# AzureLeon1/DiffSpectra

Hardware: AMD Instinct MI355X
Metric: molecules/sec, 1000-step QM9S all-spectra sampling (partial run) (higher is better)
Workload: dtype f32 (GEMMs as split-fp16 x3 MFMA with fp32 accumulate; fp32-level accuracy, parity gates unchanged)

## Files before the change

diffspectra_amd/csrc/ds_device.h:

```cpp
#pragma once
#include <hip/hip_runtime.h>
#include <stdint.h>

typedef float f32x16 __attribute__((ext_vector_type(16)));
typedef float f32x2 __attribute__((ext_vector_type(2)));
typedef _Float16 h4 __attribute__((ext_vector_type(4)));
typedef _Float16 h8 __attribute__((ext_vector_type(8)));
typedef float f32x4 __attribute__((ext_vector_type(4)));

#define DS_LDP 4

__device__ __forceinline__ float ds_silu(float x) { return __fdividef(x, 1.0f + __expf(-x)); }
__device__ __forceinline__ float ds_tanh(float x) {
  const float e = __builtin_amdgcn_exp2f(x * 2.8853900817779268f);
  return fmaf(-2.0f, __builtin_amdgcn_rcpf(e + 1.0f), 1.0f);
}
__device__ __forceinline__ f32x2 ds_tanh2_prescaled(f32x2 t) {
  f32x2 e;
  e.x = __builtin_amdgcn_exp2f(t.x); e.y = __builtin_amdgcn_exp2f(t.y);
  const f32x2 d = e + 1.0f;
  f32x2 r;
  r.x = __builtin_amdgcn_rcpf(d.x); r.y = __builtin_amdgcn_rcpf(d.y);
  return r * -2.0f + 1.0f;
}
// ... 235 lines not shown
      }
    }
    __builtin_amdgcn_sched_barrier(0);
#pragma unroll
    for (int m = 0; m < MT; ++m) {
      if (TRANS) {
        hi[m] = __builtin_amdgcn_mfma_f32_32x32x16_f16(w1, xa[m][0], hi[m], 0, 0, 0);
        lo[m] = __builtin_amdgcn_mfma_f32_32x32x16_f16(w1, xa[m][1], lo[m], 0, 0, 0);
        lo[m] = __builtin_amdgcn_mfma_f32_32x32x16_f16(w2, xa[m][0], lo[m], 0, 0, 0);
      } else {
        hi[m] = __builtin_amdgcn_mfma_f32_32x32x16_f16(xa[m][0], w1, hi[m], 0, 0, 0);
        lo[m] = __builtin_amdgcn_mfma_f32_32x32x16_f16(xa[m][1], w1, lo[m], 0, 0, 0);
        lo[m] = __builtin_amdgcn_mfma_f32_32x32x16_f16(xa[m][0], w2, lo[m], 0, 0, 0);
      }
    }
    w1 = w1n; w2 = w2n;
#pragma unroll
    for (int m = 0; m < MT; ++m) {
      if (XPF) { xa[m][0] = xn[m][0]; xa[m][1] = xn[m][1]; }
      else {
        xa[m][0] = *reinterpret_cast<const h8*>(xr + m * 32 * ldh + kn * 16);
        xa[m][1] = *reinterpret_cast<const h8*>(xr + m * 32 * ldh + K_tile + kn * 16);
      }
    }
  }
}
constexpr int DS_MMA_XD = 1;
template <int PF>
struct WRingH {
  h8 w1[PF], w2[PF];
};
template <int PF>
__device__ __forceinline__ void wring_h(WRingH<PF>& ring, const WStreamH& ws, int kb0) {
#pragma unroll
  for (int i = 0; i < PF; ++i) {
    ring.w1[i] = wload_h(ws, 0, kb0 + i); ring.w2[i] = wload_h(ws, 1, kb0 + i);
    __builtin_amdgcn_sched_barrier(0);
  }
}
template <int MT, bool TRANS, int NKB, int PF, int XD = DS_MMA_XD>
__device__ __forceinline__ void wave_mma_h_deep(const _Float16* X, int K_tile, const WStreamH& ws, WRingH<PF>& ring, int kb0,
                                                f32x16 (&hi)[MT], f32x16 (&lo)[MT], int xkb0 = 0) {
  static_assert(PF <= NKB && XD <= NKB, "ring deeper than the product");
  const int lane = threadIdx.x & 63, r = lane & 31, hh = lane >> 5;
  const int ldh = 2 * K_tile + 8;
  const _Float16* xr = X + r * ldh + 8 * hh + (kb0 - xkb0) * 16;
  h8 xq[XD][MT][2];
#pragma unroll
  for (int d = 0; d < XD; ++d)
#pragma unroll
    for (int m = 0; m < MT; ++m) {
      xq[d][m][0] = *reinterpret_cast<const h8*>(xr + m * 32 * ldh + d * 16);
      xq[d][m][1] = *reinterpret_cast<const h8*>(xr + m * 32 * ldh + K_tile + d * 16);
    }
#pragma unroll
  for (int i = 0; i < NKB; ++i) {
    __builtin_amdgcn_sched_barrier(0);
    const h8 w1 = ring.w1[i % PF], w2 = ring.w2[i % PF];
    h8 xa[MT][2];
#pragma unroll
    for (int m = 0; m < MT; ++m) { xa[m][0] = xq[i % XD][m][0]; xa[m][1] = xq[i % XD][m][1]; }
#define DS_MMA_(ACC, WV, XV) ACC = TRANS ? __builtin_amdgcn_mfma_f32_32x32x16_f16(WV, XV, ACC, 0, 0, 0) : __builtin_amdgcn_mfma_f32_32x32x16_f16(XV, WV, ACC, 0, 0, 0)
#pragma unroll
    for (int m = 0; m < MT; ++m) DS_MMA_(lo[m], w1, xa[m][1]);
#pragma unroll
    for (int m = 0; m < MT; ++m) DS_MMA_(hi[m], w1, xa[m][0]);
#pragma unroll
    for (int m = 0; m < MT; ++m) DS_MMA_(lo[m], w2, xa[m][0]);
#undef DS_MMA_
    if (i + PF < NKB) {
      ring.w1[i % PF] = wload_h(ws, 0, kb0 + i + PF);
      ring.w2[i % PF] = wload_h(ws, 1, kb0 + i + PF);
    }
    if (i + XD < NKB) {
#pragma unroll
      for (int m = 0; m < MT; ++m) {
        xq[i % XD][m][0] = *reinterpret_cast<const h8*>(xr + m * 32 * ldh + (i + XD) * 16);
        xq[i % XD][m][1] = *reinterpret_cast<const h8*>(xr + m * 32 * ldh + K_tile + (i + XD) * 16);
      }
    }
    __builtin_amdgcn_sched_barrier(0);
  }
}
template <int MT, bool TRANS, int NKB, int PF>
__device__ __forceinline__ void wave_mma_h_deep_t2(const _Float16* X, int K_tile, const WStreamH& wsA, const WStreamH& wsB,
                                                   WRingH<PF>& ringA, WRingH<PF>& ringB, int kb0, f32x16 (&hiA)[MT], f32x16 (&loA)[MT],
                                                   f32x16 (&hiB)[MT], f32x16 (&loB)[MT], int xkb0 = 0) {
  static_assert(PF <= NKB, "ring deeper than the product");
  const int lane = threadIdx.x & 63, r = lane & 31, hh = lane >> 5;
  const int ldh = 2 * K_tile + 8;
  const _Float16* xr = X + r * ldh + 8 * hh + (kb0 - xkb0) * 16;
  h8 xa[MT][2];
#pragma unroll
  for (int m = 0; m < MT; ++m) {
    xa[m][0] = *reinterpret_cast<const h8*>(xr + m * 32 * ldh);
    xa[m][1] = *reinterpret_cast<const h8*>(xr + m * 32 * ldh + K_tile);
  }
#define DS_MMA_(ACC, WV, XV) ACC = TRANS ? __builtin_amdgcn_mfma_f32_32x32x16_f16(WV, XV, ACC, 0, 0, 0) : __builtin_amdgcn_mfma_f32_32x32x16_f16(XV, WV, ACC, 0, 0, 0)
#pragma unroll
  for (int i = 0; i < NKB; ++i) {
    const int in = i + 1 < NKB ? i + 1 : i;
    h8 xn[MT][2];
#pragma unroll
    for (int m = 0; m < MT; ++m) {
      xn[m][0] = *reinterpret_cast<const h8*>(xr + m * 32 * ldh + in * 16);
      xn[m][1] = *reinterpret_cast<const h8*>(xr + m * 32 * ldh + K_tile + in * 16);
    }
    __builtin_amdgcn_sched_barrier(0);
    const h8 a1 = ringA.w1[i % PF], a2 = ringA.w2[i % PF], b1 = ringB.w1[i % PF], b2 = ringB.w2[i % PF];
#pragma unroll
    for (int m = 0; m < MT; ++m) { DS_MMA_(loA[m], a1, xa[m][1]); DS_MMA_(loB[m], b1, xa[m][1]); }
#pragma unroll
    for (int m = 0; m < MT; ++m) { DS_MMA_(hiA[m], a1, xa[m][0]); DS_MMA_(hiB[m], b1, xa[m][0]); }
#pragma unroll
    for (int m = 0; m < MT; ++m) { DS_MMA_(loA[m], a2, xa[m][0]); DS_MMA_(loB[m], b2, xa[m][0]); }
    if (i + PF < NKB) {
      ringA.w1[i % PF] = wload_h(wsA, 0, kb0 + i + PF); ringA.w2[i % PF] = wload_h(wsA, 1, kb0 + i + PF);
      ringB.w1[i % PF] = wload_h(wsB, 0, kb0 + i + PF); ringB.w2[i % PF] = wload_h(wsB, 1, kb0 + i + PF);
    }
    __builtin_amdgcn_sched_barrier(0);
#pragma unroll
    for (int m = 0; m < MT; ++m) { xa[m][0] = xn[m][0]; xa[m][1] = xn[m][1]; }
  }
#undef DS_MMA_
}
template <int MT, bool TRANS, int NKB, int PF>
__device__ __forceinline__ void wave_mma_h_ring_t2(const _Float16* X, int K_tile, const WStreamH& wsA, const WStreamH& wsB, int kb0,
                                                   f32x16 (&hiA)[MT], f32x16 (&loA)[MT], f32x16 (&hiB)[MT], f32x16 (&loB)[MT], int xkb0 = 0) {
  WRingH<PF> ringA, ringB;
#pragma unroll
  for (int i = 0; i < PF; ++i) {
    ringA.w1[i] = wload_h(wsA, 0, kb0 + i); ringA.w2[i] = wload_h(wsA, 1, kb0 + i);
    ringB.w1[i] = wload_h(wsB, 0, kb0 + i); ringB.w2[i] = wload_h(wsB, 1, kb0 + i);
    __builtin_amdgcn_sched_barrier(0);
  }
  wave_mma_h_deep_t2<MT, TRANS, NKB, PF>(X, K_tile, wsA, wsB, ringA, ringB, kb0, hiA, loA, hiB, loB, xkb0);
}

template <int MT, bool TRANS, int NKB, int PF>
__device__ __forceinline__ void wave_mma_h_ring(const _Float16* X, int K_tile, const float* __restrict__ Wh, int N, int K, int col0,
                                                int kb0, f32x16 (&hi)[MT], f32x16 (&lo)[MT], int xkb0 = 0) {
  const WStreamH ws = wstream_h(Wh, N, K, col0);
  WRingH<PF> ring;
  wring_h<PF>(ring, ws, kb0);
  wave_mma_h_deep<MT, TRANS, NKB, PF>(X, K_tile, ws, ring, kb0, hi, lo, xkb0);
}
template <int MT>
__device__ __forceinline__ void split_finish(f32x16 (&hi)[MT], const f32x16 (&lo)[MT]) {
#pragma unroll
  for (int m = 0; m < MT; ++m)
#pragma unroll
    for (int i = 0; i < 16; ++i) hi[m][i] = fmaf(lo[m][i], 1.0f / 2048.0f, hi[m][i]);
}

template <int MT>
__device__ __forceinline__ void acc_zero(f32x16 (&acc)[MT]) {
#pragma unroll
  for (int m = 0; m < MT; ++m)
#pragma unroll
    for (int i = 0; i < 16; ++i) acc[m][i] = 0.0f;
}

template <int MT, class F>
__device__ __forceinline__ void acc_foreach(const f32x16 (&acc)[MT], int row_base, int col0, F f) {
  const int lane = threadIdx.x & 63, r = lane & 31, hh = lane >> 5;
#pragma unroll
  for (int m = 0; m < MT; ++m)
#pragma unroll
    for (int i = 0; i < 16; ++i) f(row_base + m * 32 + acc_row(i, hh), col0 + r, acc[m][i]);
}

struct RowStore {
  __amdgpu_buffer_rsrc_t rsrc;
  int voff;
};
template <int LD>
__device__ __forceinline__ RowStore row_store(float* dst) {
  const int lane = threadIdx.x & 63;
  const unsigned long long pw = reinterpret_cast<unsigned long long>(dst);
  const unsigned long long pu = (static_cast<unsigned long long>(__builtin_amdgcn_readfirstlane(static_cast<int>(pw >> 32))) << 32) |
                                static_cast<unsigned int>(__builtin_amdgcn_readfirstlane(static_cast<int>(pw)));
  RowStore s;
  s.rsrc = __builtin_amdgcn_make_buffer_rsrc(reinterpret_cast<float*>(pu), 0, 0x7fffffff, 0x00020000);
  s.voff = ((4 * (lane >> 5)) * LD + (lane & 31)) * 4;
  return s;
}
__device__ __forceinline__ void row_put(const RowStore& s, int row_byte_off, float v) {
  __builtin_amdgcn_raw_buffer_store_b32(__float_as_uint(v), s.rsrc, s.voff, row_byte_off, 0);
}
template <int MT, int LD, class F>
__device__ __forceinline__ void acc_store(const f32x16 (&acc)[MT], float* __restrict__ dst, int rows_valid, F f) {
  const int lane = threadIdx.x & 63, r = lane & 31, hh = lane >> 5;
  const RowStore st = row_store<LD>(dst);
  if (rows_valid >= 32 * MT) {
#pragma unroll
    for (int m = 0; m < MT; ++m)
#pragma unroll
      for (int i = 0; i < 16; ++i) row_put(st, (m * 32 + (i & 3) + 8 * (i >> 2)) * LD * 4, f(r, acc[m][i]));
  } else {
// ... 52 lines not shown
```

diffspectra_amd/csrc/ds_forward.hip:

```cpp
#include <hip/hip_runtime.h>
#include <math.h>
#include <stdint.h>
#include <stdlib.h>

#include <atomic>
#include <mutex>
#include <utility>
#include <vector>

#include "../../include/diffspectra_hip.h"
#include "../../include/diffspectra_step.h"
#include "../../include/diffspectra_tiles.h"
#include "ds_device.h"
#include "ds_host.h"

#define ADAC DS_ADA_COLS
constexpr int DS_NODE_PF = 8;
constexpr int DS_NODE_PF2 = 4;
constexpr int DS_QKV_PF = 4;
constexpr int DS_QKV_PF_WIDE = 4;
constexpr int DS_NODE_TILE64_MIN_PER_CU = 4;
constexpr int DS_TWO_STREAM_MAX_PAIRS = 400000;

#ifdef DS_STAMPS
// ... 1502 lines not shown
#pragma unroll
          for (int u = 0; u < 4; ++u) {
            const float4 e = reinterpret_cast<const float4*>(&Xh[buf][2 * q][0])[16 * u + j];
            x[u].x = (Ka[u].x + Bv[bt][u].x) + e.x; x[u].y = (Ka[u].y + Bv[bt][u].y) + e.y;
            x[u].z = (Ka[u].z + Bv[bt][u].z) + e.z; x[u].w = (Ka[u].w + Bv[bt][u].w) + e.w;
          }
          __builtin_amdgcn_sched_barrier(0);
          if (have_next) DS_EQUI_ISSUE_B(bt, bv_x);
          if (bt + 1 < NPASS) DS_EQUI_ISSUE_A(bt + 1);
          __builtin_amdgcn_sched_barrier(0);
          DS_STAMP(12);
          ln_mod_quad256(x, sh, sc);
          _Float16* xr = &Xh[buf][2 * q + gdir][0];
#pragma unroll
          for (int u = 0; u < 4; ++u) split_store4(xr, 256, 64 * u + 4 * j, x[u]);
          if (bt + 1 < NPASS) DS_EQUI_ISSUE_M(bt + 1);
          DS_STAMP(14);
        }
        if (npairs < TP) {
          for (int i = 0; i < PPW; ++i) {
            const int qz = lw * PPW + i;
            if (qz >= npairs) {
              float4* z = reinterpret_cast<float4*>(&Xh[buf][2 * qz][0]);
              z[lane] = make_float4(0, 0, 0, 0);
              z[64 + lane] = make_float4(0, 0, 0, 0);
              if (lane < 2) z[128 + lane] = make_float4(0, 0, 0, 0);
            }
          }
        }
      }
      DS_STAMP(7);
      __syncthreads();
      DS_STAMP(9);
      if (!have) break;
      pv_c = pv_x; av_c = av_x; bv_c = bv_x; mv_c = mv_x; adj_c = adj_x;
      if (tile + 2 * stride < ntiles) DS_EQUI_FETCH_IDX(tile + 2 * stride, pv_x, av_x, bv_x, mv_x, adj_x);
    }
#undef DS_EQUI_FETCH_IDX
#undef DS_EQUI_ISSUE_B
#undef DS_EQUI_ISSUE_A
#undef DS_EQUI_ISSUE_M
    DS_STAMP_FLUSH(NCW * 64);
  }
}

__global__ __launch_bounds__(64) void k_pos_update(Ctx c, int last) {
  const int m = blockIdx.x, r = threadIdx.x;
  const int n0 = c.L.node_off[m], n = c.L.node_off[m + 1] - n0;
  const int p0 = c.L.pair_off[m];
  if (n <= 0) return;
  float x = 0.0f, y = 0.0f, z = 0.0f;
  if (r < n) {
    const float4* tr = reinterpret_cast<const float4*>(c.ws.tr);
    float sx = 0.0f, sy = 0.0f, sz = 0.0f;
    for (int c0 = 0; c0 < n; c0 += 8) {
      float4 t[8];
#pragma unroll
      for (int u = 0; u < 8; ++u) {
        const int cc = c0 + u;
        t[u] = make_float4(0, 0, 0, 0);
        if (cc < n && cc != r) {
          const int lo = r < cc ? r : cc, hi = r < cc ? cc : r;
          const int pl = lo * (2 * n - lo - 1) / 2 + (hi - lo - 1);
          t[u] = tr[(size_t)(p0 + pl) * 2 + (r < cc ? 0 : 1)];
        }
      }
#pragma unroll
      for (int u = 0; u < 8; ++u)
        if (c0 + u < n && c0 + u != r) { sx += t[u].x; sy += t[u].y; sz += t[u].z; }
    }
    const float* pp = c.ws.pos + (size_t)(n0 + r) * 4;
    x = pp[0] + sx; y = pp[1] + sy; z = pp[2] + sz;
  }
  const float fn = (float)n;
  const float mx = wave_sum(x) / fn, my = wave_sum(y) / fn, mz = wave_sum(z) / fn;
  if (r < n) {
    float* pp = c.ws.pos + (size_t)(n0 + r) * 4;
    const float ox = x - mx, oy = y - my, oz = z - mz;
    pp[0] = ox; pp[1] = oy; pp[2] = oz;
    if (last && (isnan(ox) || isnan(oy) || isnan(oz))) atomicOr(&c.ws.flags[1], 1);
  }
}

__global__ __launch_bounds__(256) void k_node_readout(Ctx c, float* __restrict__ out_xh) {
  ds_fp16_saturate();
  constexpr int T = 32;
  __shared__ __attribute__((aligned(16))) _Float16 X[T][2 * 768 + 8];
  __shared__ __attribute__((aligned(16))) _Float16 Y1[T][2 * 256 + 8];
  __shared__ __attribute__((aligned(16))) float Y2[T][128 + DS_LDP];
  __shared__ int dn[T];
  const int tid = threadIdx.x, wave = tid >> 6, row0 = blockIdx.x * T;
  const int Nn = c.L.Nn;
  if (tid < T) dn[tid] = row0 + tid < Nn ? c.L.node_dense[row0 + tid] : -1;
  for (int i0 = tid; i0 < T * 192; i0 += 256 * 8) {
    float4 v[8];
#pragma unroll
    for (int u = 0; u < 8; ++u) {
      const int idx = i0 + u * 256, row = idx / 192, k4 = idx - row * 192;
      v[u] = reinterpret_cast<const float4*>(c.ws.atom_hids + (size_t)min(row0 + row, Nn - 1) * 768)[k4];
    }
#pragma unroll
    for (int u = 0; u < 8; ++u) {
      const int idx = i0 + u * 256, row = idx / 192, k4 = idx - row * 192;
      split_store4(&X[row][0], 768, 4 * k4, row0 + row < Nn ? v[u] : make_float4(0, 0, 0, 0));
    }
  }
  __syncthreads();
  {
    const float* b = GW(c, DS_GW_NP0_B);
    for (int ch = wave; ch < 8; ch += 4) {
      asm volatile("" ::: "memory");
      const int col = ch * 32 + (tid & 31), hhf = (tid & 63) >> 5;
      const float bc = b[col];
      f32x16 acc[1], lo[1];
#pragma unroll
      for (int i = 0; i < 16; ++i) acc[0][i] = bc;
      acc_zero<1>(lo);
      wave_mma_h_ring<1, false, 48, 8>(&X[0][0], 768, GW(c, DS_GW_NP0_H), 256, 768, ch * 32, 0, acc, lo);
      split_finish<1>(acc, lo);
#pragma unroll
      for (int i = 0; i < 16; ++i) split_store1(&Y1[acc_row(i, hhf)][0], 256, col, ds_silu(acc[0][i]));
    }
  }
  __syncthreads();
  {
    const float* b = GW(c, DS_GW_NP2_B);
    const int col = wave * 32 + (tid & 31), hhf = (tid & 63) >> 5;
    const float bc = b[col];
    f32x16 acc[1], lo[1];
#pragma unroll
    for (int i = 0; i < 16; ++i) acc[0][i] = bc;
    acc_zero<1>(lo);
    wave_mma_h_ring<1, false, 16, 8>(&Y1[0][0], 256, GW(c, DS_GW_NP2_H), 128, 256, wave * 32, 0, acc, lo);
    split_finish<1>(acc, lo);
#pragma unroll
    for (int i = 0; i < 16; ++i) Y2[acc_row(i, hhf)][col] = ds_silu(acc[0][i]);
  }
  __syncthreads();
  {
    const float* b = GW(c, DS_GW_NP4_B);
    const float bc = b[min((int)(threadIdx.x & 31), 5)];
    tile_gemm<1, 1>(&Y2[0][0], 128 + DS_LDP, 128, GW(c, DS_GW_NP4_W), 32, 1, [&](int row, int col, float v) {
      if (col < 6 && dn[row] >= 0) out_xh[(size_t)dn[row] * 9 + 3 + col] = v + bc;
    });
  }
}

__global__ __launch_bounds__(256) void k_edge_readout(Ctx c, float* __restrict__ out_edge) {
  ds_fp16_saturate();
  const int tid = threadIdx.x, wave = tid >> 6, lane = tid & 63, r = lane & 31, hh = lane >> 5;
  const int Pp = c.L.Pp;
  const int row0 = (blockIdx.x * 4 + wave) * 32;
  if (row0 >= Pp) return;
  const int p = min(row0 + r, Pp - 1);
  const bool valid = row0 + r < Pp;
  const int pa = c.L.pair_a[p], pb = c.L.pair_b[p], pm = c.L.pair_mol[p];
  h8 x1[12], x2[12];
  {
    const float4* src = reinterpret_cast<const float4*>(c.ws.edge_hids + (size_t)p * 192 + 8 * hh);
#pragma unroll
    for (int g4 = 0; g4 < 3; ++g4) {
      float4 v[4][2];
#pragma unroll
      for (int u = 0; u < 4; ++u) { v[u][0] = src[(g4 * 4 + u) * 4]; v[u][1] = src[(g4 * 4 + u) * 4 + 1]; }
#pragma unroll
      for (int u = 0; u < 4; ++u) {
        const float xs[8] = {v[u][0].x, v[u][0].y, v[u][0].z, v[u][0].w, v[u][1].x, v[u][1].y, v[u][1].z, v[u][1].w};
#pragma unroll
        for (int t = 0; t < 8; ++t) {
          const _Float16 a1 = (_Float16)xs[t];
          x1[g4 * 4 + u][t] = a1;
          x2[g4 * 4 + u][t] = (_Float16)((xs[t] - (float)a1) * 2048.0f);
        }
      }
    }
  }
  const int da = c.L.node_dense[pa], db = c.L.node_dense[pb];
  const int mN = pm * c.L.N;
  const size_t oab = ((size_t)da * c.L.N + (db - mN)) * 2, oba = ((size_t)db * c.L.N + (da - mN)) * 2;
  for (int ch = 0; ch < 2; ++ch) {
    const int g0 = ch == 0 ? DS_GW_EX0_W : DS_GW_ET0_W;
    const float* b0 = GW(c, g0 + 1);
    const float* b2 = GW(c, g0 + 3);
    const uint4* W2 = reinterpret_cast<const uint4*>(GW(c, ch == 0 ? DS_GW_EX2_C : DS_GW_ET2_C)) + lane;
    f32x16 a2, a2lo;
#pragma unroll
    for (int q = 0; q < 4; ++q) {
      const float4 bb = *reinterpret_cast<const float4*>(b2 + 8 * q + 4 * hh);
      a2[4 * q] = bb.x; a2[4 * q + 1] = bb.y; a2[4 * q + 2] = bb.z; a2[4 * q + 3] = bb.w;
    }
#pragma unroll
    for (int i = 0; i < 16; ++i) a2lo[i] = 0.0f;
#pragma unroll
    for (int hc = 0; hc < 2; ++hc) {
      asm volatile("" ::: "memory");
      const WStreamH ws0 = wstream_h(GW(c, ch == 0 ? DS_GW_EX0_H : DS_GW_ET0_H), 64, 192, hc * 32);
      WRingH<6> ring;
      wring_h<6>(ring, ws0, 0);
      f32x16 a1, a1lo;
#pragma unroll
      for (int q = 0; q < 4; ++q) {
        const float4 bb = *reinterpret_cast<const float4*>(b0 + hc * 32 + 8 * q + 4 * hh);
        a1[4 * q] = bb.x; a1[4 * q + 1] = bb.y; a1[4 * q + 2] = bb.z; a1[4 * q + 3] = bb.w;
      }
#pragma unroll
      for (int i = 0; i < 16; ++i) a1lo[i] = 0.0f;
#pragma unroll
      for (int kb = 0; kb < 12; ++kb) {
        const h8 w1 = ring.w1[kb % 6], w2 = ring.w2[kb % 6];
        a1lo = __builtin_amdgcn_mfma_f32_32x32x16_f16(w1, x2[kb], a1lo, 0, 0, 0);
        a1 = __builtin_amdgcn_mfma_f32_32x32x16_f16(w1, x1[kb], a1, 0, 0, 0);
        a1lo = __builtin_amdgcn_mfma_f32_32x32x16_f16(w2, x1[kb], a1lo, 0, 0, 0);
        if (kb + 6 < 12) { ring.w1[kb % 6] = wload_h(ws0, 0, kb + 6); ring.w2[kb % 6] = wload_h(ws0, 1, kb + 6); }
        __builtin_amdgcn_sched_barrier(0);
      }
#pragma unroll
      for (int i = 0; i < 16; ++i) a1[i] = fmaf(a1lo[i], 1.0f / 2048.0f, a1[i]);
#pragma unroll
      for (int s_ = 0; s_ < 2; ++s_) {
        h8 y1, y2;
#pragma unroll
        for (int j = 0; j < 8; j += 2) {
          f32x2 v;
          v.x = a1[8 * s_ + j]; v.y = a1[8 * s_ + j + 1];
          v = ds_silu2(v);
          y1[j] = (_Float16)v.x; y1[j + 1] = (_Float16)v.y;
          y2[j] = (_Float16)((v.x - (float)y1[j]) * 2048.0f); y2[j + 1] = (_Float16)((v.y - (float)y1[j + 1]) * 2048.0f);
        }
        const h8 w1 = __builtin_bit_cast(h8, W2[((0 * 2 + hc) * 2 + s_) * 64]);
        const h8 w2 = __builtin_bit_cast(h8, W2[((1 * 2 + hc) * 2 + s_) * 64]);
        a2 = __builtin_amdgcn_mfma_f32_32x32x16_f16(w1, y1, a2, 0, 0, 0);
        a2lo = __builtin_amdgcn_mfma_f32_32x32x16_f16(w1, y2, a2lo, 0, 0, 0);
        a2lo = __builtin_amdgcn_mfma_f32_32x32x16_f16(w2, y1, a2lo, 0, 0, 0);
      }
    }
    const float* W4 = GW(c, g0 + 4);
    f32x2 s2 = {0.0f, 0.0f};
#pragma unroll
    for (int i = 0; i < 16; i += 2) {
      f32x2 v;
      v.x = fmaf(a2lo[i], 1.0f / 2048.0f, a2[i]); v.y = fmaf(a2lo[i + 1], 1.0f / 2048.0f, a2[i + 1]);
      v = ds_silu2(v);
      const f32x2 w = {wp_at(W4, 32, acc_row(i, hh), 0), wp_at(W4, 32, acc_row(i + 1, hh), 0)};
      s2 = __builtin_elementwise_fma(w, v, s2);
    }
    const float part = s2.x + s2.y;
    const auto sw = __builtin_amdgcn_permlane32_swap(__float_as_uint(part), __float_as_uint(part), false, false);
    const float val = (__uint_as_float(sw[0]) + __uint_as_float(sw[1])) + GW(c, g0 + 5)[0];
    if (valid && hh == 0) {
      out_edge[oab + ch] = val;
      out_edge[oba + ch] = val;
    }
  }
}

__global__ void k_final_pos(Ctx c, float* __restrict__ out_xh) {
  const int m = blockIdx.x * blockDim.x + threadIdx.x;
  if (m >= c.L.B) return;
  const int n0 = c.L.node_off[m], n = c.L.node_off[m + 1] - n0;
  const bool nan = c.ws.flags[1] != 0;
  float sx = 0.0f, sy = 0.0f, sz = 0.0f;
  for (int a = 0; a < n; ++a) {
    const float* pp = c.ws.pos + (size_t)(n0 + a) * 4;
    if (!nan) { sx += pp[0]; sy += pp[1]; sz += pp[2]; }
  }
  const float fn = (float)n;
  for (int a = 0; a < n; ++a) {
    const float* pp = c.ws.pos + (size_t)(n0 + a) * 4;
    float* o = out_xh + (size_t)c.L.node_dense[n0 + a] * 9;
    const float px = nan ? 0.0f : pp[0], py = nan ? 0.0f : pp[1], pz = nan ? 0.0f : pp[2];
    o[0] = px - sx / fn; o[1] = py - sy / fn; o[2] = pz - sz / fn;
  }
}

__global__ void k_temb_finish(Ctx c, const float* __restrict__ tm3, int tm3_rows, const float* __restrict__ ctx) {
  ds_fp16_saturate();
  const size_t i = (size_t)blockIdx.x * blockDim.x + threadIdx.x;
  if (i >= (size_t)c.L.B * 1024) return;
  const size_t b = i >> 10, col = i & 1023;
  float v = tm3[(tm3_rows == 1 ? 0 : b) * 1024 + col];
  if (ctx) v += ctx[i];
  split_store1(reinterpret_cast<_Float16*>(c.ws.temb_silu) + b * 2048, 1024, (int)col, ds_silu(v));
}

bool make_ctx(Ctx& c, const ds_weights* w, const ds_layout* L, const ds_workspace* ws) {
  if (!w || !L || !ws || !w->base || !w->off_dev) return false;
  if (L->max_n > DS_MAX_ATOMS || L->B <= 0) return false;
  c.L = *L; c.ws = *ws; c.wbase = w->base; c.woff = w->off_dev;
  c.edge_th = w->edge_th; c.cutoff = w->spatial_cut_off;
  return true;
}

constexpr int MAX_DEVICES = 16;

inline int device_cus() {
  static std::atomic<int> cus[MAX_DEVICES];
  int dev = 0, n = 0;
  if (hipGetDevice(&dev) != hipSuccess || dev < 0 || dev >= MAX_DEVICES) return 256;
  if ((n = cus[dev].load(std::memory_order_relaxed)) > 0) return n;
  if (hipDeviceGetAttribute(&n, hipDeviceAttributeMultiprocessorCount, dev) != hipSuccess || n <= 0) n = 256;
  cus[dev].store(n, std::memory_order_relaxed);
  return n;
}

enum ProfSlot { PROF_EDGE_GEOM = 0, PROF_NODE_QKV = 1, PROF_ATTN = 2, PROF_NODE_UPDATE = 3, PROF_EDGE_UPDATE = 4, PROF_EQUI_PAIRS = 5 };
struct ProfState {
  int kernel = -1;
  int every = 1;
  long long seen = 0;
  std::vector<std::pair<hipEvent_t, hipEvent_t>> pool;
  size_t used = 0;
};
ProfState g_prof;

struct ProfScope {
  hipStream_t s;
  bool on = false;
  ProfScope(int kernel, hipStream_t st) : s(st) {
    if (g_prof.kernel != kernel) return;
    if ((g_prof.seen++ % g_prof.every) != 0 || g_prof.used >= g_prof.pool.size()) return;
    on = true;
    (void)hipEventRecord(g_prof.pool[g_prof.used].first, s);
  }
  ~ProfScope() {
    if (on) (void)hipEventRecord(g_prof.pool[g_prof.used++].second, s);
  }
};

void launch_edge_geom(const Ctx& c, int blk, hipStream_t s) {
  if (c.L.Pp <= 0) return;
  ProfScope ps(PROF_EDGE_GEOM, s);
  hipLaunchKernelGGL(k_edge_geom, dim3((c.L.Pp + 63) / 64), dim3(256), 0, s, c, blk);
}
int g_node_tile = -1;
bool node_tile64(const Ctx& c) {
  static const int env_tile = [] { const char* e = getenv("DIFFSPECTRA_NODE_TILE"); return e ? atoi(e) : -1; }();
// ... 27 lines not shown
  ProfScope ps(PROF_EQUI_PAIRS, s);
  hipLaunchKernelGGL(k_equi_pairs, dim3(min((c.L.Pp + 31) / 32, device_cus())), dim3((EQUI_NCW + EQUI_NLW) * 64), 0, s, c, blk);
}
void launch_pos_update(const Ctx& c, int last, hipStream_t s) { hipLaunchKernelGGL(k_pos_update, dim3(c.L.B), dim3(64), 0, s, c, last); }

}

extern "C" {

void ds_struct_sizes(int64_t* out) {
  out[0] = sizeof(ds_weights);
  out[1] = sizeof(ds_layout);
  out[2] = sizeof(ds_workspace);
  out[3] = sizeof(ds_gemm_args);
}

static int stage_time(const ds_weights* w, const ds_layout* L, ds_workspace* ws, const float* noise_level, const float* ctx_emb,
                      int rows, void* stream) {
  hipStream_t s = (hipStream_t)stream;
  Ctx c;
  if (!make_ctx(c, w, L, ws) || !noise_level) return DS_ERR_ARG;
  const int B = L->B;
  const int64_t* off = w->off + DS_NBLOCKS * DS_W_BLOCK_SLOTS;
  hipLaunchKernelGGL(k_time_feat, dim3((rows + 63) / 64), dim3(64), 0, s, c, noise_level, rows);
  ds_gemm_args g{};
  g.A = ws->tfeat; g.lda = 24; g.Wp = w->base + off[DS_GW_TM1_W]; g.bias = w->base + off[DS_GW_TM1_B];
  g.C = ws->tmid; g.ldc = 1024; g.M = rows; g.K = 24; g.N = 1024; g.act = 2;
  int st = dst::gemm_routed_as(&g, B, stream);
  if (st) return st;
  float* tm3 = ws->ada;
  g.A = ws->tmid; g.lda = 1024; g.Wp = w->base + off[DS_GW_TM3_W]; g.bias = w->base + off[DS_GW_TM3_B];
  g.C = tm3; g.K = 1024; g.act = 0;
  st = dst::gemm_routed_as(&g, B, stream);
  if (st) return st;
  const size_t tot = (size_t)B * 1024;
  hipLaunchKernelGGL(k_temb_finish, dim3((unsigned)((tot + 255) / 256)), dim3(256), 0, s, c, (const float*)tm3, rows, ctx_emb);
  static_assert(ADAC % 32 == 0, "adaLN table width");
  return ds_gemm_split(ws->temb_silu, w->base + off[DS_GW_ADA_W], w->base + off[DS_GW_ADA_B], ws->ada, ADAC, B, 1024, ADAC, stream);
}

int ds_stage_time(const ds_weights* w, const ds_layout* L, ds_workspace* ws, const float* noise_level, const float* ctx_emb,
                  void* stream) {
  return L ? stage_time(w, L, ws, noise_level, ctx_emb, L->B, stream) : DS_ERR_ARG;
}

int ds_stage_time_uniform(const ds_weights* w, const ds_layout* L, ds_workspace* ws, const float* noise_level, const float* ctx_emb,
                          void* stream) {
  return stage_time(w, L, ws, noise_level, ctx_emb, 1, stream);
}

int ds_stage_init(const ds_weights* w, const ds_layout* L, ds_workspace* ws, const float* xh, const float* edge_x,
                  const float* cond_x, const float* cond_edge_x, void* stream) {
  hipStream_t s = (hipStream_t)stream;
  Ctx c;
  if (!make_ctx(c, w, L, ws) || !xh || !edge_x || ((cond_x == nullptr) != (cond_edge_x == nullptr))) return DS_ERR_ARG;
  if (!clear(ws->flags, 8 * sizeof(int32_t), s)) return DS_ERR_LAUNCH;
  if (L->Pp > 0) hipLaunchKernelGGL(k_pair_flags, dim3((L->Pp + 1023) / 1024), dim3(1024), 0, s, c, cond_x, cond_edge_x);
  hipLaunchKernelGGL(k_node_init, dim3((L->Nn + 7) / 8), dim3(256), 0, s, c, xh, cond_x);
  if (L->Pp > 0) hipLaunchKernelGGL(k_pair_init, dim3((L->Pp + 63) / 64), dim3(256), 0, s, c, edge_x, cond_x, cond_edge_x);
  return DST_CHECK_LAUNCH();
}

int ds_stage_block(const ds_weights* w, const ds_layout* L, ds_workspace* ws, int blk, int last, void* stream) {
  hipStream_t s = (hipStream_t)stream;
  Ctx c;
  if (!make_ctx(c, w, L, ws) || blk < 0 || blk >= DS_NBLOCKS) return DS_ERR_ARG;
  launch_edge_geom(c, blk, s);
  launch_node_qkv(c, blk, s);
  launch_attn(c, blk, s);
  launch_node_update<true>(c, blk, s);
  launch_edge_update(c, blk, s);
  launch_equi_pairs(c, blk, s);
  launch_pos_update(c, last, s);
  return DST_CHECK_LAUNCH();
}

int ds_stage_readout(const ds_weights* w, const ds_layout* L, ds_workspace* ws, float* out_xh, float* out_edge, void* stream) {
  hipStream_t s = (hipStream_t)stream;
  Ctx c;
  if (!make_ctx(c, w, L, ws) || !out_xh || !out_edge) return DS_ERR_ARG;
  const size_t nx = (size_t)L->B * L->N * 9, ne = (size_t)L->B * L->N * L->N * 2;
  if (!clear(out_xh, nx * sizeof(float), s) || !clear(out_edge, ne * sizeof(float), s)) return DS_ERR_LAUNCH;
  hipLaunchKernelGGL(k_node_readout, dim3((L->Nn + 31) / 32), dim3(256), 0, s, c, out_xh);
  if (L->Pp > 0) hipLaunchKernelGGL(k_edge_readout, dim3((L->Pp + 127) / 128), dim3(256), 0, s, c, out_edge);
  hipLaunchKernelGGL(k_final_pos, dim3((L->B + 63) / 64), dim3(64), 0, s, c, out_xh);
  return DST_CHECK_LAUNCH();
}

struct SideStream {
  hipStream_t s = nullptr;
  hipEvent_t fork[DS_NBLOCKS + 1] = {}, join[DS_NBLOCKS + 1] = {};
  std::once_flag once;
  bool ok = false;
};
static SideStream g_side[MAX_DEVICES];
static int g_two_stream = -1;

static SideStream* side_stream() {
  int dev = 0;
  if (hipGetDevice(&dev) != hipSuccess || dev < 0 || dev >= MAX_DEVICES) return nullptr;
  SideStream& ss = g_side[dev];
  std::call_once(ss.once, [&ss] {
    bool ok = hipStreamCreateWithFlags(&ss.s, hipStreamNonBlocking) == hipSuccess;
    for (int i = 0; ok && i <= DS_NBLOCKS; ++i)
      ok = hipEventCreateWithFlags(&ss.fork[i], hipEventDisableTiming) == hipSuccess &&
           hipEventCreateWithFlags(&ss.join[i], hipEventDisableTiming) == hipSuccess;
    ss.ok = ok;
  });
  return ss.ok ? &ss : nullptr;
}

static int forward_blocks_two_streams(const ds_weights* w, const ds_layout* L, ds_workspace* ws, hipStream_t s, SideStream* ss) {
  Ctx c;
  if (!make_ctx(c, w, L, ws)) return DS_ERR_ARG;
  hipStream_t s2 = ss->s;
  const hipEvent_t fork0 = ss->fork[DS_NBLOCKS], join0 = ss->join[DS_NBLOCKS];
  if (!record(fork0, s) || !wait(s2, fork0)) return DS_ERR_LAUNCH;
  launch_node_qkv(c, 0, s2);
  if (!record(join0, s2)) return DS_ERR_LAUNCH;
  for (int blk = 0; blk < DS_NBLOCKS; ++blk) {
    launch_edge_geom(c, blk, s);
    if (!wait(s, blk == 0 ? join0 : ss->join[blk - 1])) return DS_ERR_LAUNCH;
    launch_attn(c, blk, s);
    launch_node_n2e(c, blk, s);
    if (!record(ss->fork[blk], s) || !wait(s2, ss->fork[blk])) return DS_ERR_LAUNCH;
    launch_node_update<false>(c, blk, s2);
    if (blk + 1 < DS_NBLOCKS) launch_node_qkv(c, blk + 1, s2);
    if (!record(ss->join[blk], s2)) return DS_ERR_LAUNCH;
    launch_edge_update(c, blk, s);
    if (!wait(s, ss->join[blk])) return DS_ERR_LAUNCH;
    launch_equi_pairs(c, blk, s);
    launch_pos_update(c, blk == DS_NBLOCKS - 1 ? 1 : 0, s);
  }
  return DST_CHECK_LAUNCH();
}

int ds_set_two_stream(int on) {
  const int prev = g_two_stream;
  g_two_stream = on;
  return prev;
}

int ds_set_node_tile(int rows) {
  const int prev = g_node_tile;
  g_node_tile = (rows == 32 || rows == 64) ? rows : -1;
  return prev;
}

static int forward(const ds_weights* w, const ds_layout* L, ds_workspace* ws, const float* xh, const float* edge_x, const float* cond_x,
                   const float* cond_edge_x, const float* noise_level, const float* ctx_emb, float* out_xh, float* out_edge,
                   bool uniform, void* stream) {
  int st = uniform ? ds_stage_time_uniform(w, L, ws, noise_level, ctx_emb, stream) : ds_stage_time(w, L, ws, noise_level, ctx_emb, stream);
  if (st) return st;
  st = ds_stage_init(w, L, ws, xh, edge_x, cond_x, cond_edge_x, stream);
  if (st) return st;
  static const int env_two = [] { const char* e = getenv("DIFFSPECTRA_TWO_STREAM"); return e ? atoi(e) : -1; }();
  const int pick = g_two_stream >= 0 ? g_two_stream : env_two;
  const int two = pick >= 0 ? pick : (L->Pp < DS_TWO_STREAM_MAX_PAIRS ? 1 : 0);
  SideStream* ss = two ? side_stream() : nullptr;
  if (ss) {
    st = forward_blocks_two_streams(w, L, ws, (hipStream_t)stream, ss);
    if (st) return st;
  } else {
    for (int b = 0; b < DS_NBLOCKS; ++b) {
      st = ds_stage_block(w, L, ws, b, b == DS_NBLOCKS - 1, stream);
      if (st) return st;
    }
// ... 45 lines not shown
```

Before: 237.9.

## Stream node readout input in K-chunks and make edge readout persistent with LDS weights

Node readout now stages atom_hids in double-buffered 128-wide K chunks, overlapping global loads with the MFMA loop. Each wave computes two column tiles at once through a continued weight ring, and Y1 overlays the X ring to cut shared memory so three blocks can fit per CU. Edge readout becomes a persistent grid-stride kernel with 8 waves that copies both heads' weights and biases into LDS once per block and prefetches the next tile's edge features during the current tile's MFMAs. The cost is more register pressure and added complexity, and only the final readout stage is affected.

Result: no change. 239.3 (median of 6 runs) (+0.6%).

```diff
diff --git a/diffspectra_amd/csrc/ds_device.h b/diffspectra_amd/csrc/ds_device.h
--- a/diffspectra_amd/csrc/ds_device.h
+++ b/diffspectra_amd/csrc/ds_device.h
@@ -341,11 +341,12 @@
     __builtin_amdgcn_sched_barrier(0);
   }
 }
-template <int MT, bool TRANS, int NKB, int PF>
+template <int MT, bool TRANS, int NKB, int PF, bool CONT = false>
 __device__ __forceinline__ void wave_mma_h_deep_t2(const _Float16* X, int K_tile, const WStreamH& wsA, const WStreamH& wsB,
                                                    WRingH<PF>& ringA, WRingH<PF>& ringB, int kb0, f32x16 (&hiA)[MT], f32x16 (&loA)[MT],
-                                                   f32x16 (&hiB)[MT], f32x16 (&loB)[MT], int xkb0 = 0) {
+                                                   f32x16 (&hiB)[MT], f32x16 (&loB)[MT], int xkb0 = 0, int kb_end = 0) {
   static_assert(PF <= NKB, "ring deeper than the product");
+  static_assert(!CONT || NKB % PF == 0, "a continued ring keeps block kb in slot kb % PF");
   const int lane = threadIdx.x & 63, r = lane & 31, hh = lane >> 5;
   const int ldh = 2 * K_tile + 8;
   const _Float16* xr = X + r * ldh + 8 * hh + (kb0 - xkb0) * 16;
@@ -373,7 +374,7 @@
     for (int m = 0; m < MT; ++m) { DS_MMA_(hiA[m], a1, xa[m][0]); DS_MMA_(hiB[m], b1, xa[m][0]); }
 #pragma unroll
     for (int m = 0; m < MT; ++m) { DS_MMA_(loA[m], a2, xa[m][0]); DS_MMA_(loB[m], b2, xa[m][0]); }
-    if (i + PF < NKB) {
+    if (i + PF < NKB || (CONT && kb0 + i + PF < kb_end)) {
       ringA.w1[i % PF] = wload_h(wsA, 0, kb0 + i + PF); ringA.w2[i % PF] = wload_h(wsA, 1, kb0 + i + PF);
       ringB.w1[i % PF] = wload_h(wsB, 0, kb0 + i + PF); ringB.w2[i % PF] = wload_h(wsB, 1, kb0 + i + PF);
     }
diff --git a/diffspectra_amd/csrc/ds_forward.hip b/diffspectra_amd/csrc/ds_forward.hip
--- a/diffspectra_amd/csrc/ds_forward.hip
+++ b/diffspectra_amd/csrc/ds_forward.hip
@@ -1608,45 +1608,67 @@
   }
 }
 
-__global__ __launch_bounds__(256) void k_node_readout(Ctx c, float* __restrict__ out_xh) {
+constexpr int DS_NR_KC = 128;
+__global__ __launch_bounds__(256, 3) void k_node_readout(Ctx c, float* __restrict__ out_xh) {
   ds_fp16_saturate();
-  constexpr int T = 32;
-  __shared__ __attribute__((aligned(16))) _Float16 X[T][2 * 768 + 8];
-  __shared__ __attribute__((aligned(16))) _Float16 Y1[T][2 * 256 + 8];
+  constexpr int T = 32, KC = DS_NR_KC, NC = 768 / KC, KBC = KC / 16, PF = 2;
+  constexpr int XROW = 2 * KC + 8, Y1ROW = 2 * 256 + 8;
+  constexpr int RING = 2 * T * XROW;
+  static_assert(768 % KC == 0 && RING >= T * Y1ROW, "Y1 overlays the X ring");
+  __shared__ __attribute__((aligned(16))) _Float16 XY[RING];
   __shared__ __attribute__((aligned(16))) float Y2[T][128 + DS_LDP];
   __shared__ int dn[T];
+  _Float16 (*const Xc)[T][XROW] = reinterpret_cast<_Float16 (*)[T][XROW]>(XY);
+  _Float16 (*const Y1)[Y1ROW] = reinterpret_cast<_Float16 (*)[Y1ROW]>(XY);
   const int tid = threadIdx.x, wave = tid >> 6, row0 = blockIdx.x * T;
   const int Nn = c.L.Nn;
   if (tid < T) dn[tid] = row0 + tid < Nn ? c.L.node_dense[row0 + tid] : -1;
-  for (int i0 = tid; i0 < T * 192; i0 += 256 * 8) {
-    float4 v[8];
-#pragma unroll
-    for (int u = 0; u < 8; ++u) {
-      const int idx = i0 + u * 256, row = idx / 192, k4 = idx - row * 192;
-      v[u] = reinterpret_cast<const float4*>(c.ws.atom_hids + (size_t)min(row0 + row, Nn - 1) * 768)[k4];
-    }
-#pragma unroll
-    for (int u = 0; u < 8; ++u) {
-      const int idx = i0 + u * 256, row = idx / 192, k4 = idx - row * 192;
-      split_store4(&X[row][0], 768, 4 * k4, row0 + row < Nn ? v[u] : make_float4(0, 0, 0, 0));
-    }
-  }
-  __syncthreads();
-  {
+  const int k4 = tid & 31, srow = tid >> 5;
+  const float4* src = reinterpret_cast<const float4*>(c.ws.atom_hids) + k4;
+  float4 v[4];
+  auto fetch = [&](int ck) {
+#pragma unroll
+    for (int u = 0; u < 4; ++u) v[u] = src[(size_t)min(row0 + srow + 8 * u, Nn - 1) * 192 + ck * (KC / 4)];
+  };
+  auto stash = [&](int buf) {
+#pragma unroll
+    for (int u = 0; u < 4; ++u)
+      split_store4(&Xc[buf][srow + 8 * u][0], KC, 4 * k4, row0 + srow + 8 * u < Nn ? v[u] : make_float4(0, 0, 0, 0));
+  };
+  fetch(0);
+  {
+    const int col = wave * 32 + (tid & 31), hhf = (tid & 63) >> 5;
+    const WStreamH wsA = wstream_h(GW(c, DS_GW_NP0_H), 256, 768, wave * 32), wsB = wstream_h(GW(c, DS_GW_NP0_H), 256, 768, (wave + 4) * 32);
+    WRingH<PF> ringA, ringB;
+#pragma unroll
+    for (int i = 0; i < PF; ++i) {
+      ringA.w1[i] = wload_h(wsA, 0, i); ringA.w2[i] = wload_h(wsA, 1, i);
+      ringB.w1[i] = wload_h(wsB, 0, i); ringB.w2[i] = wload_h(wsB, 1, i);
+      __builtin_amdgcn_sched_barrier(0);
+    }
     const float* b = GW(c, DS_GW_NP0_B);
-    for (int ch = wave; ch < 8; ch += 4) {
-      asm volatile("" ::: "memory");
-      const int col = ch * 32 + (tid & 31), hhf = (tid & 63) >> 5;
-      const float bc = b[col];
-      f32x16 acc[1], lo[1];
-#pragma unroll
-      for (int i = 0; i < 16; ++i) acc[0][i] = bc;
-      acc_zero<1>(lo);
-      wave_mma_h_ring<1, false, 48, 8>(&X[0][0], 768, GW(c, DS_GW_NP0_H), 256, 768, ch * 32, 0, acc, lo);
-      split_finish<1>(acc, lo);
-#pragma unroll
-      for (int i = 0; i < 16; ++i) split_store1(&Y1[acc_row(i, hhf)][0], 256, col, ds_silu(acc[0][i]));
-    }
+    const float bcA = b[col], bcB = b[col + 128];
+    f32x16 accA[1], loA[1], accB[1], loB[1];
+#pragma unroll
+    for (int i = 0; i < 16; ++i) { accA[0][i] = bcA; accB[0][i] = bcB; }
+    acc_zero<1>(loA);
+    acc_zero<1>(loB);
+    stash(0);
+    fetch(1);
+    __syncthreads();
+#pragma unroll
+    for (int ck = 0; ck < NC; ++ck) {
+      wave_mma_h_deep_t2<1, false, KBC, PF, true>(&Xc[ck & 1][0][0], KC, wsA, wsB, ringA, ringB, ck * KBC, accA, loA, accB, loB, ck * KBC, 48);
+      if (ck + 1 < NC) stash((ck + 1) & 1);
+      if (ck + 2 < NC) fetch(ck + 2);
+      __syncthreads();
+    }
+    split_finish<1>(accA, loA);
+    split_finish<1>(accB, loB);
+#pragma unroll
+    for (int i = 0; i < 16; ++i) split_store1(&Y1[acc_row(i, hhf)][0], 256, col, ds_silu(accA[0][i]));
+#pragma unroll
+    for (int i = 0; i < 16; ++i) split_store1(&Y1[acc_row(i, hhf)][0], 256, col + 128, ds_silu(accB[0][i]));
   }
   __syncthreads();
   {
@@ -1672,112 +1694,142 @@
   }
 }
 
-__global__ __launch_bounds__(256) void k_edge_readout(Ctx c, float* __restrict__ out_edge) {
+constexpr int DS_ER_WAVES = 8;
+constexpr int DS_ER_W0_U4 = 2 * 12 * 2 * 64;
+constexpr int DS_ER_W2_U4 = 2 * 2 * 2 * 64;
+__global__ __launch_bounds__(DS_ER_WAVES * 64) void k_edge_readout(Ctx c, float* __restrict__ out_edge) {
   ds_fp16_saturate();
+  __shared__ uint4 W0s[2][DS_ER_W0_U4];
+  __shared__ uint4 W2s[2][DS_ER_W2_U4];
+  __shared__ __attribute__((aligned(16))) float B0s[2][64], B2s[2][32], W4s[2][32];
+  __shared__ float B4s[2];
   const int tid = threadIdx.x, wave = tid >> 6, lane = tid & 63, r = lane & 31, hh = lane >> 5;
-  const int Pp = c.L.Pp;
-  const int row0 = (blockIdx.x * 4 + wave) * 32;
-  if (row0 >= Pp) return;
-  const int p = min(row0 + r, Pp - 1);
-  const bool valid = row0 + r < Pp;
-  const int pa = c.L.pair_a[p], pb = c.L.pair_b[p], pm = c.L.pair_mol[p];
-  h8 x1[12], x2[12];
-  {
+  const int Pp = c.L.Pp, ntiles = (Pp + 31) / 32, tstride = gridDim.x * DS_ER_WAVES;
+  int tile = blockIdx.x * DS_ER_WAVES + wave;
+  float4 xr[12][2];
+  int pa, pb, pm;
+  {
+    const int p = min(tile * 32 + r, Pp - 1);
     const float4* src = reinterpret_cast<const float4*>(c.ws.edge_hids + (size_t)p * 192 + 8 * hh);
 #pragma unroll
-    for (int g4 = 0; g4 < 3; ++g4) {
-      float4 v[4][2];
-#pragma unroll
-      for (int u = 0; u < 4; ++u) { v[u][0] = src[(g4 * 4 + u) * 4]; v[u][1] = src[(g4 * 4 + u) * 4 + 1]; }
-#pragma unroll
-      for (int u = 0; u < 4; ++u) {
-        const float xs[8] = {v[u][0].x, v[u][0].y, v[u][0].z, v[u][0].w, v[u][1].x, v[u][1].y, v[u][1].z, v[u][1].w};
-#pragma unroll
-        for (int t = 0; t < 8; ++t) {
-          const _Float16 a1 = (_Float16)xs[t];
-          x1[g4 * 4 + u][t] = a1;
-          x2[g4 * 4 + u][t] = (_Float16)((xs[t] - (float)a1) * 2048.0f);
-        }
-      }
-    }
-  }
-  const int da = c.L.node_dense[pa], db = c.L.node_dense[pb];
-  const int mN = pm * c.L.N;
-  const size_t oab = ((size_t)da * c.L.N + (db - mN)) * 2, oba = ((size_t)db * c.L.N + (da - mN)) * 2;
+    for (int kb = 0; kb < 12; ++kb) { xr[kb][0] = src[kb * 4]; xr[kb][1] = src[kb * 4 + 1]; }
+    pa = c.L.pair_a[p]; pb = c.L.pair_b[p]; pm = c.L.pair_mol[p];
+  }
+#pragma unroll
   for (int ch = 0; ch < 2; ++ch) {
     const int g0 = ch == 0 ? DS_GW_EX0_W : DS_GW_ET0_W;
-    const float* b0 = GW(c, g0 + 1);
-    const float* b2 = GW(c, g0 + 3);
-    const uint4* W2 = reinterpret_cast<const uint4*>(GW(c, ch == 0 ? DS_GW_EX2_C : DS_GW_ET2_C)) + lane;
-    f32x16 a2, a2lo;
-#pragma unroll
-    for (int q = 0; q < 4; ++q) {
-      const float4 bb = *reinterpret_cast<const float4*>(b2 + 8 * q + 4 * hh);
-      a2[4 * q] = bb.x; a2[4 * q + 1] = bb.y; a2[4 * q + 2] = bb.z; a2[4 * q + 3] = bb.w;
-    }
-#pragma unroll
-    for (int i = 0; i < 16; ++i) a2lo[i] = 0.0f;
-#pragma unroll
-    for (int hc = 0; hc < 2; ++hc) {
-      asm volatile("" ::: "memory");
-      const WStreamH ws0 = wstream_h(GW(c, ch == 0 ? DS_GW_EX0_H : DS_GW_ET0_H), 64, 192, hc * 32);
-      WRingH<6> ring;
-      wring_h<6>(ring, ws0, 0);
-      f32x16 a1, a1lo;
+    const uint4* w0 = reinterpret_cast<const uint4*>(GW(c, ch == 0 ? DS_GW_EX0_H : DS_GW_ET0_H));
+    const uint4* w2 = reinterpret_cast<const uint4*>(GW(c, ch == 0 ? DS_GW_EX2_C : DS_GW_ET2_C));
+#pragma unroll
+    for (int i = 0; i < DS_ER_W0_U4 / (DS_ER_WAVES * 64); ++i) W0s[ch][i * DS_ER_WAVES * 64 + tid] = w0[i * DS_ER_WAVES * 64 + tid];
+    W2s[ch][tid] = w2[tid];
+    if (tid < 64) B0s[ch][tid] = GW(c, g0 + 1)[tid];
+    else if (tid < 96) B2s[ch][tid - 64] = GW(c, g0 + 3)[tid - 64];
+    else if (tid < 128) W4s[ch][tid - 96] = wp_at(GW(c, g0 + 4), 32, tid - 96, 0);
+    else if (tid == 128) B4s[ch] = GW(c, g0 + 5)[0];
+  }
+  static_assert(DS_ER_W0_U4 % (DS_ER_WAVES * 64) == 0 && DS_ER_W2_U4 == DS_ER_WAVES * 64, "weight copy: whole trips of the workgroup");
+  __syncthreads();
+  const int wl = hh * 64 + r;
+#define DS_ER_W(S, PL) __builtin_bit_cast(h8, W0s[(S) / 24][(PL) * 1536 + ((S) % 12) * 128 + (((S) / 12) & 1) * 32 + wl])
+  h8 rw1[2], rw2[2];
+  rw1[0] = DS_ER_W(0, 0); rw2[0] = DS_ER_W(0, 1);
+  rw1[1] = DS_ER_W(1, 0); rw2[1] = DS_ER_W(1, 1);
+  for (; tile < ntiles; tile += tstride) {
+    const int row0 = tile * 32;
+    const bool valid = row0 + r < Pp;
+    int da = c.L.node_dense[pa], db = c.L.node_dense[pb];
+    const int mN = pm * c.L.N;
+    const int pn = min((tile + tstride) * 32 + r, Pp - 1);
+    pa = c.L.pair_a[pn]; pb = c.L.pair_b[pn]; pm = c.L.pair_mol[pn];
+    const float4* nsrc = reinterpret_cast<const float4*>(c.ws.edge_hids + (size_t)pn * 192 + 8 * hh);
+    h8 x1[12], x2[12];
+    auto split = [&](int kb) {
+      const float xs[8] = {xr[kb][0].x, xr[kb][0].y, xr[kb][0].z, xr[kb][0].w, xr[kb][1].x, xr[kb][1].y, xr[kb][1].z, xr[kb][1].w};
+#pragma unroll
+      for (int t = 0; t < 8; ++t) {
+        const _Float16 a1 = (_Float16)xs[t];
+        x1[kb][t] = a1;
+        x2[kb][t] = (_Float16)((xs[t] - (float)a1) * 2048.0f);
+      }
+    };
+    split(0);
+    size_t oab = 0, oba = 0;
+#pragma unroll
+    for (int ch = 0; ch < 2; ++ch) {
+      f32x16 a2, a2lo;
 #pragma unroll
       for (int q = 0; q < 4; ++q) {
-        const float4 bb = *reinterpret_cast<const float4*>(b0 + hc * 32 + 8 * q + 4 * hh);
-        a1[4 * q] = bb.x; a1[4 * q + 1] = bb.y; a1[4 * q + 2] = bb.z; a1[4 * q + 3] = bb.w;
-      }
-#pragma unroll
-      for (int i = 0; i < 16; ++i) a1lo[i] = 0.0f;
-#pragma unroll
-      for (int kb = 0; kb < 12; ++kb) {
-        const h8 w1 = ring.w1[kb % 6], w2 = ring.w2[kb % 6];
-        a1lo = __builtin_amdgcn_mfma_f32_32x32x16_f16(w1, x2[kb], a1lo, 0, 0, 0);
-        a1 = __builtin_amdgcn_mfma_f32_32x32x16_f16(w1, x1[kb], a1, 0, 0, 0);
-        a1lo = __builtin_amdgcn_mfma_f32_32x32x16_f16(w2, x1[kb], a1lo, 0, 0, 0);
-        if (kb + 6 < 12) { ring.w1[kb % 6] = wload_h(ws0, 0, kb + 6); ring.w2[kb % 6] = wload_h(ws0, 1, kb + 6); }
-        __builtin_amdgcn_sched_barrier(0);
-      }
-#pragma unroll
-      for (int i = 0; i < 16; ++i) a1[i] = fmaf(a1lo[i], 1.0f / 2048.0f, a1[i]);
-#pragma unroll
-      for (int s_ = 0; s_ < 2; ++s_) {
-        h8 y1, y2;
-#pragma unroll
-        for (int j = 0; j < 8; j += 2) {
-          f32x2 v;
-          v.x = a1[8 * s_ + j]; v.y = a1[8 * s_ + j + 1];
-          v = ds_silu2(v);
-          y1[j] = (_Float16)v.x; y1[j + 1] = (_Float16)v.y;
-          y2[j] = (_Float16)((v.x - (float)y1[j]) * 2048.0f); y2[j + 1] = (_Float16)((v.y - (float)y1[j + 1]) * 2048.0f);
+        const float4 bb = *reinterpret_cast<const float4*>(&B2s[ch][8 * q + 4 * hh]);
+        a2[4 * q] = bb.x; a2[4 * q + 1] = bb.y; a2[4 * q + 2] = bb.z; a2[4 * q + 3] = bb.w;
+      }
+#pragma unroll
+      for (int i = 0; i < 16; ++i) a2lo[i] = 0.0f;
+#pragma unroll
+      for (int hc = 0; hc < 2; ++hc) {
+        f32x16 a1, a1lo;
+#pragma unroll
+        for (int q = 0; q < 4; ++q) {
+          const float4 bb = *reinterpret_cast<const float4*>(&B0s[ch][hc * 32 + 8 * q + 4 * hh]);
+          a1[4 * q] = bb.x; a1[4 * q + 1] = bb.y; a1[4 * q + 2] = bb.z; a1[4 * q + 3] = bb.w;
         }
-        const h8 w1 = __builtin_bit_cast(h8, W2[((0 * 2 + hc) * 2 + s_) * 64]);
-        const h8 w2 = __builtin_bit_cast(h8, W2[((1 * 2 + hc) * 2 + s_) * 64]);
-        a2 = __builtin_amdgcn_mfma_f32_32x32x16_f16(w1, y1, a2, 0, 0, 0);
-        a2lo = __builtin_amdgcn_mfma_f32_32x32x16_f16(w1, y2, a2lo, 0, 0, 0);
-        a2lo = __builtin_amdgcn_mfma_f32_32x32x16_f16(w2, y1, a2lo, 0, 0, 0);
-      }
-    }
-    const float* W4 = GW(c, g0 + 4);
-    f32x2 s2 = {0.0f, 0.0f};
-#pragma unroll
-    for (int i = 0; i < 16; i += 2) {
-      f32x2 v;
-      v.x = fmaf(a2lo[i], 1.0f / 2048.0f, a2[i]); v.y = fmaf(a2lo[i + 1], 1.0f / 2048.0f, a2[i + 1]);
-      v = ds_silu2(v);
-      const f32x2 w = {wp_at(W4, 32, acc_row(i, hh), 0), wp_at(W4, 32, acc_row(i + 1, hh), 0)};
-      s2 = __builtin_elementwise_fma(w, v, s2);
-    }
-    const float part = s2.x + s2.y;
-    const auto sw = __builtin_amdgcn_permlane32_swap(__float_as_uint(part), __float_as_uint(part), false, false);
-    const float val = (__uint_as_float(sw[0]) + __uint_as_float(sw[1])) + GW(c, g0 + 5)[0];
-    if (valid && hh == 0) {
-      out_edge[oab + ch] = val;
-      out_edge[oba + ch] = val;
-    }
-  }
+#pragma unroll
+        for (int i = 0; i < 16; ++i) a1lo[i] = 0.0f;
+#pragma unroll
+        for (int kb = 0; kb < 12; ++kb) {
+          const int s_ = (ch * 2 + hc) * 12 + kb;
+          if (ch == 0 && hc == 0 && kb + 1 < 12) split(kb + 1);
+          const h8 w1 = rw1[s_ % 2], w2 = rw2[s_ % 2];
+          a1lo = __builtin_amdgcn_mfma_f32_32x32x16_f16(w1, x2[kb], a1lo, 0, 0, 0);
+          a1 = __builtin_amdgcn_mfma_f32_32x32x16_f16(w1, x1[kb], a1, 0, 0, 0);
+          a1lo = __builtin_amdgcn_mfma_f32_32x32x16_f16(w2, x1[kb], a1lo, 0, 0, 0);
+          rw1[s_ % 2] = DS_ER_W((s_ + 2) % 48, 0); rw2[s_ % 2] = DS_ER_W((s_ + 2) % 48, 1);
+          if (ch == 1 && hc == 1) { xr[kb][0] = nsrc[kb * 4]; xr[kb][1] = nsrc[kb * 4 + 1]; }
+          __builtin_amdgcn_sched_barrier(0);
+        }
+#pragma unroll
+        for (int i = 0; i < 16; ++i) a1[i] = fmaf(a1lo[i], 1.0f / 2048.0f, a1[i]);
+#pragma unroll
+        for (int s_ = 0; s_ < 2; ++s_) {
+          h8 y1, y2;
+#pragma unroll
+          for (int j = 0; j < 8; j += 2) {
+            f32x2 v;
+            v.x = a1[8 * s_ + j]; v.y = a1[8 * s_ + j + 1];
+            v = ds_silu2(v);
+            y1[j] = (_Float16)v.x; y1[j + 1] = (_Float16)v.y;
+            y2[j] = (_Float16)((v.x - (float)y1[j]) * 2048.0f); y2[j + 1] = (_Float16)((v.y - (float)y1[j + 1]) * 2048.0f);
+          }
+          const h8 w1 = __builtin_bit_cast(h8, W2s[ch][((0 * 2 + hc) * 2 + s_) * 64 + lane]);
+          const h8 w2 = __builtin_bit_cast(h8, W2s[ch][((1 * 2 + hc) * 2 + s_) * 64 + lane]);
+          a2 = __builtin_amdgcn_mfma_f32_32x32x16_f16(w1, y1, a2, 0, 0, 0);
+          a2lo = __builtin_amdgcn_mfma_f32_32x32x16_f16(w1, y2, a2lo, 0, 0, 0);
+          a2lo = __builtin_amdgcn_mfma_f32_32x32x16_f16(w2, y1, a2lo, 0, 0, 0);
+        }
+      }
+      if (ch == 0) {
+        asm volatile("" : "+v"(da), "+v"(db));
+        oab = ((size_t)da * c.L.N + (db - mN)) * 2; oba = ((size_t)db * c.L.N + (da - mN)) * 2;
+      }
+      f32x2 s2 = {0.0f, 0.0f};
+#pragma unroll
+      for (int i = 0; i < 16; i += 2) {
+        f32x2 v;
+        v.x = fmaf(a2lo[i], 1.0f / 2048.0f, a2[i]); v.y = fmaf(a2lo[i + 1], 1.0f / 2048.0f, a2[i + 1]);
+        v = ds_silu2(v);
+        const f32x2 w = {W4s[ch][acc_row(i, hh)], W4s[ch][acc_row(i + 1, hh)]};
+        s2 = __builtin_elementwise_fma(w, v, s2);
+      }
+      const float part = s2.x + s2.y;
+      const auto sw = __builtin_amdgcn_permlane32_swap(__float_as_uint(part), __float_as_uint(part), false, false);
+      const float val = (__uint_as_float(sw[0]) + __uint_as_float(sw[1])) + B4s[ch];
+      if (valid && hh == 0) {
+        out_edge[oab + ch] = val;
+        out_edge[oba + ch] = val;
+      }
+    }
+  }
+#undef DS_ER_W
 }
 
 __global__ void k_final_pos(Ctx c, float* __restrict__ out_xh) {
@@ -1971,7 +2023,8 @@
   const size_t nx = (size_t)L->B * L->N * 9, ne = (size_t)L->B * L->N * L->N * 2;
   if (!clear(out_xh, nx * sizeof(float), s) || !clear(out_edge, ne * sizeof(float), s)) return DS_ERR_LAUNCH;
   hipLaunchKernelGGL(k_node_readout, dim3((L->Nn + 31) / 32), dim3(256), 0, s, c, out_xh);
-  if (L->Pp > 0) hipLaunchKernelGGL(k_edge_readout, dim3((L->Pp + 127) / 128), dim3(256), 0, s, c, out_edge);
+  if (L->Pp > 0)
+    hipLaunchKernelGGL(k_edge_readout, dim3(min((L->Pp + 32 * DS_ER_WAVES - 1) / (32 * DS_ER_WAVES), device_cus())), dim3(DS_ER_WAVES * 64), 0, s, c, out_edge);
   hipLaunchKernelGGL(k_final_pos, dim3((L->B + 63) / 64), dim3(64), 0, s, c, out_xh);
   return DST_CHECK_LAUNCH();
 }
```
